# adelacvg/detail_tts

Measured on AMD Instinct MI355X. Metric: generated audio seconds/sec (24 kHz), 10 s prompt, batch 8 per GPU, higher is better.
Workload: dtype f32; 1 GPU; configs[2]: 1xMI355X batch-8, 10 s prompts (T_ref=936), 234 codes -> 9.984 s audio per utterance; GPT KV-cache decode + 50-step CFG diffusion + flow-VAE/HiFiGAN vocoder, seed-0 random-init weights; batch_per_gpu=8, codes=234, diffusion_steps=50, parallelism=replica x1

## Files before the change

detail_tts_amd/csrc/conv_gemm.h:

```cpp
#pragma once
#include "common.h"

namespace dtts {

struct ConvParams {
    const float* x = nullptr;
    long long x_bs = 0;
    int x_cs = 0;
    const int* len_in = nullptr;
    const int* x_bidx = nullptr;
    int Tin = 0;
    const float* pro_ab = nullptr;
    int pro_act = ACT_NONE;
    float pro_slope = 0.f;
    const float* w = nullptr;
    const float* bias = nullptr;
    int Cin = 0, CinP = 0, Cout = 0, CoutP = 0, KW = 1, stride = 1, dil = 1, pad = 0;
    const float* badd = nullptr;
    int badd_bs = 0;
    int gate = GATE_NONE;
    int epi_act = ACT_NONE;
    float epi_slope = 0.f;
    float out_scale = 1.f;
    const float* res = nullptr;
// ... 22 lines not shown
    int gn_ada_stride = 0;
    const int* gn_ada_idx = nullptr;
    int gn_act = ACT_NONE, gn_groups = 32;
    float gn_eps = 1e-5f;
    void* gn_xch = nullptr;
    unsigned gn_tag = 0;
    int* gn_err = nullptr;
    const int* cols = nullptr;
    int ncols = 0, cols_b0 = 0;
    void* next3 = nullptr;
    int next_c8 = 0, next_tp = 0, next_halo = 0, next_act = ACT_NONE;
    float next_slope = 0.f;
    int* next_sat = nullptr;
    int ksplit = 1;
    int ksplit_max = 0;
    int p1 = 0;
    int epi_vec = 0;
    float* kpart = nullptr;
    int* kcount = nullptr;
    int ablate = 0;
};

void launch_conv_gemm(const ConvParams& p, hipStream_t stream);
void set_conv_small_tiles(int n);

}
```

detail_tts_amd/csrc/conv_gemm.hip:

```cpp
#include <atomic>
#include <cstdlib>
#include "conv_gemm_kernel.h"

namespace dtts {

static int conv_small_tiles_default() {
    static const int n = env_int("DTTS_CONV_SMALL_TILES", 384);
    return n;
}
static std::atomic<int> g_conv_small_tiles{-1};
void set_conv_small_tiles(int n) { g_conv_small_tiles.store(n < 0 ? -1 : n, std::memory_order_relaxed); }

void launch_conv_gemm(const ConvParams& p_in, hipStream_t stream) {
    static const int ablate = env_int("DTTS_CONV_ABLATE", 0);
    ConvParams p = p_in;
    p.ablate = ablate;
    DTTS_REQUIRE(p.B > 0 && p.Nout > 0 && p.Cout > 0 && p.Cin > 0, "empty conv");
    DTTS_REQUIRE(p.x && p.w && p.y, "null pointer");
    DTTS_REQUIRE(p.gate == GATE_NONE || p.phases == 1, "gate+phases unsupported");
    const int halo = (p.KW - 1) * p.dil;
    auto fits = [&](int bn) { return (bn - 1) * p.stride + halo + 1 <= XW_MAX; };
    const int small_opt = g_conv_small_tiles.load(std::memory_order_relaxed);
    const int small_tiles = small_opt >= 0 ? small_opt : conv_small_tiles_default();
    if (small_tiles > 0 && p.CoutP % 64 == 0 && fits(64) && (long long)cdiv(p.CoutP, 128) * cdiv(p.Nout, 128) * p.B <= small_tiles) {
        static const int small_bk = env_int("DTTS_CONV_SMALL_BK", 32);
        if (small_bk == 32 && p.CinP % 32 == 0 && p.KW * p.dil <= 3) launch_conv_tile<64, 64, 2, 2, 32>(p, stream, "conv_gemm_kernel<64,64,k32>");
        else launch_conv_tile<64, 64, 2, 2, 16>(p, stream, "conv_gemm_kernel<64,64,k16>");
        return;
    }
    if (p.CoutP % 128 == 0) {
        const int pad128 = round_up(p.Nout, 128), pad64 = round_up(p.Nout, 64);
        if (fits(128) && (pad128 - pad64) * 10 <= p.Nout) {
            launch_conv_tile<128, 128, 2, 2, 16>(p, stream, "conv_gemm_kernel<128,128,k16>");
        } else {
            DTTS_REQUIRE(fits(64), "conv halo too large");
            launch_conv_tile<128, 64, 2, 2, 16>(p, stream, "conv_gemm_kernel<128,64,k16>");
        }
    } else if (p.CoutP % 64 == 0) {
        if (fits(128) && p.Nout > 64) launch_conv_tile<64, 128, 2, 2, 16>(p, stream, "conv_gemm_kernel<64,128,k16>");
// ... 10 lines not shown
```

detail_tts_amd/csrc/conv_x3.h:

```cpp
#pragma once
#include "conv_gemm.h"

namespace dtts {

constexpr int X3_HALO = 1;
constexpr int X3_BN = 192;
static inline int x3_tp(int T) { return round_up(T, X3_BN) + 2 * X3_HALO; }
static inline size_t x3_bytes(int B, int C, int T) { return (size_t)B * (C / 8) * 2 * x3_tp(T) * 16; }

void launch_split_weights(const float* wp, int KW, int CinP, int CoutP, void* out, hipStream_t s);
void launch_split_planes(const float* x, long long x_bs, int x_cs, const float* ab, int act, const int* lens, int T, int B, int C,
                         void* out, hipStream_t s);
void launch_split_planes_taps(const float* x, long long x_bs, int x_cs, const int* lens, int T, int B, int C, int KW, int pad, void* out,
                              hipStream_t s, int* sat = nullptr);
void launch_gn_split_planes(const float* x, long long x_bs, int x_cs, const int* lens, int T, int B, int C, int groups,
                            const float* gamma, const float* beta, float eps, const float* ada, int ada_stride, int ada_bs, int act,
                            void* out, hipStream_t s, const int* ada_idx = nullptr);
void launch_conv_x3(const ConvParams& p, hipStream_t s);

constexpr size_t X3_SLAB_FLOATS = 96 * 256, X3_MAX_SLABS = 1024, X3_SPLIT_COUNTERS = 4096;
void x3_split_workspace(hipStream_t s, size_t nslabs, float** part, int** count);

constexpr int GN_FUSE_MAX_NT = 6;
size_t conv_x3_gn_xch_bytes(int B, int Cout, int T);
bool conv_x3_gn_fusable(int Cout, int CoutP, int Cin, int KW, int groups, int B, int T);

constexpr int X3D_HALO = 32;
static inline int x3d_tp(int T) { return round_up(T, X3_BN) + 64 + X3D_HALO; }
static inline size_t x3d_bytes(int B, int CP, int T) { return (size_t)B * (CP / 8) * 2 * x3d_tp(T) * 16; }
void launch_split_planes_ex(const float* x, long long x_bs, int x_cs, int act, float slope, const int* lens, int T, int B, int C, int CP,
                            int halo, int Tp, void* out, hipStream_t s, int* sat = nullptr);
void launch_conv_x3d(const ConvParams& p, hipStream_t s);
void launch_zero_plane_margins(const int* lens, int T, int B, int CP, int halo, int Tp, void* out, hipStream_t s);
// ... 3 lines not shown
```

detail_tts_amd/csrc/conv_x3.hip:

```cpp
#include <algorithm>
#include <cstdio>
#include <mutex>
#include <type_traits>
#include <utility>
#include <vector>

#include "conv_x3.h"
#include <cstdlib>
#include "prof.h"
#include "split3.h"

namespace dtts {

typedef float f32x16 __attribute__((ext_vector_type(16)));

namespace {
constexpr int NPL = XS_PLANES, NK = 2 * NPL;
constexpr int BM = 128, BN = X3_BN;
constexpr int WTILE = NK * BM * 16;
constexpr int XMAIN = NK * BN * 16;
constexpr int XBUF = XMAIN + NK * 2 * 16;
typedef unsigned gn_u4 __attribute__((ext_vector_type(4)));
constexpr int GN_AUX_SC1 = 16;
constexpr int GN_MAXW = 8;
// ... 37 lines not shown
        }
#pragma unroll
        for (int e = 0; e < 8; ++e) v[e] *= XS_SCALE_X;
        split8(v, q0, q1);
    }
    uint4* o = out + ((long long)(b * C8 + c8) * NPL) * Tp + tp;
    o[0] = q0;
    o[Tp] = q1;
}

template <int ACT>
__global__ __launch_bounds__(1024) void gn_split_planes_kernel(const float* __restrict__ x, long long x_bs, int x_cs,
                                                              const int* __restrict__ lens, int T, int C, int groups,
                                                              const float* __restrict__ gamma, const float* __restrict__ beta, float eps,
                                                              const float* __restrict__ ada, int ada_stride, int ada_bs, int Tp,
                                                              uint4* __restrict__ out, const int* __restrict__ ada_idx) {
    __shared__ float red[2][16];
    __shared__ float sa[64], sd[64];
    const int g = blockIdx.x, b = blockIdx.y, tid = threadIdx.x, lane = tid & 63, wave = tid >> 6, nthr = blockDim.x;
    const int len = lens ? lens[b] : T;
    const int cpg = C / groups;
    const float* xg = x + (long long)b * x_bs + (long long)(g * cpg) * x_cs;
    const float k = xg[0];
    float s1 = 0.f, s2 = 0.f;
    const bool vec = ((x_cs & 3) == 0) && ((reinterpret_cast<unsigned long long>(xg) & 15ull) == 0);
    if (vec) {
        const int len4 = len >> 2, n4 = cpg * len4;
        for (int i0 = tid; i0 < n4; i0 += 4 * nthr) {
            float4 v[4];
#pragma unroll
            for (int u = 0; u < 4; ++u) {
                const int i = i0 + u * nthr, ic = i < n4 ? i : 0;
                const int row = ic / len4, t4 = ic - row * len4;
                v[u] = reinterpret_cast<const float4*>(xg + (long long)row * x_cs)[t4];
            }
#pragma unroll
            for (int u = 0; u < 4; ++u) {
// ... 61 lines not shown
                v[e] *= XS_SCALE_X;
            }
            split8(v, q0, q1);
        }
        uint4* o = out + ((long long)(b * C8 + g * c8n + c8l) * NPL) * Tp + tp;
        o[0] = q0;
        o[Tp] = q1;
    }
}

template <int ACT, int NI>
__global__ __launch_bounds__(1024) void gn_split_planes_reg_kernel(const float* __restrict__ x, long long x_bs, int x_cs,
                                                                  const int* __restrict__ lens, int T, int C, int groups,
                                                                  const float* __restrict__ gamma, const float* __restrict__ beta, float eps,
                                                                  const float* __restrict__ ada, int ada_stride, int ada_bs, int Tp,
                                                                  uint4* __restrict__ out, const int* __restrict__ ada_idx) {
    __shared__ float red[2][16];
    __shared__ float sa[64], sd[64];
    const int g = blockIdx.x, b = blockIdx.y, tid = threadIdx.x, lane = tid & 63, wave = tid >> 6;
    const int len = lens ? lens[b] : T;
    const int cpg = C / groups, c8n = cpg >> 3, C8 = C >> 3, nitems = c8n * Tp;
    const float* xg = x + (long long)b * x_bs + (long long)(g * cpg) * x_cs;
    const float k = xg[0];
    float v[NI][8];
    float s1 = 0.f, s2 = 0.f;
#pragma unroll
    for (int q = 0; q < NI; ++q) {
        const int item = tid + q * 1024, c8l = item / Tp, t = item - c8l * Tp - X3_HALO;
        const bool ok = item < nitems && t >= 0 && t < len;
        const float* xr = xg + (long long)(ok ? c8l * 8 : 0) * x_cs + (ok ? t : 0);
#pragma unroll
        for (int e = 0; e < 8; ++e) v[q][e] = xr[(long long)e * x_cs];
        if (ok) {
            float d[8];
#pragma unroll
            for (int e = 0; e < 8; ++e) d[e] = v[q][e] - k;
            s1 += ((d[0] + d[1]) + (d[2] + d[3])) + ((d[4] + d[5]) + (d[6] + d[7]));
// ... 846 lines not shown
    uint4* o = static_cast<uint4*>(out);
    const double n = (double)B * C * T;
    ProfScope ps("split_planes_kernel", 0.0, n * 8.0, s);
    if (ab) {
        if (act == ACT_SILU) hipLaunchKernelGGL((split_planes_kernel<ACT_SILU, true>), grid, dim3(256), 0, s, x, x_bs, x_cs, ab, lens, T, C / 8, Tp, o);
        else hipLaunchKernelGGL((split_planes_kernel<ACT_NONE, true>), grid, dim3(256), 0, s, x, x_bs, x_cs, ab, lens, T, C / 8, Tp, o);
    } else {
        if (act == ACT_SILU) hipLaunchKernelGGL((split_planes_kernel<ACT_SILU, false>), grid, dim3(256), 0, s, x, x_bs, x_cs, ab, lens, T, C / 8, Tp, o);
        else hipLaunchKernelGGL((split_planes_kernel<ACT_NONE, false>), grid, dim3(256), 0, s, x, x_bs, x_cs, ab, lens, T, C / 8, Tp, o);
    }
    DTTS_CHECK_HIP(hipGetLastError());
}

void launch_gn_split_planes(const float* x, long long x_bs, int x_cs, const int* lens, int T, int B, int C, int groups,
                            const float* gamma, const float* beta, float eps, const float* ada, int ada_stride, int ada_bs, int act,
                            void* out, hipStream_t s, const int* ada_idx) {
    DTTS_REQUIRE(C % groups == 0 && (C / groups) % 8 == 0 && C / groups <= 64, "gn_split_planes: group size");
    DTTS_REQUIRE(act == ACT_NONE || act == ACT_SILU, "gn_split_planes: activation");
    const int Tp = x3_tp(T);
    uint4* o = static_cast<uint4*>(out);
    ProfScope ps("gn_split_planes_kernel", 0.0, (double)B * C * T * 8.0, s);
    static const int ns = env_int("DTTS_GN_SPLIT_NS", 1);
    static const int nt = env_int("DTTS_GN_SPLIT_NT", 1024);
    static const bool reg_ok = env_on("DTTS_GN_SPLIT_REG");
    constexpr int NI = 3;
    if (reg_ok && ns == 1 && (C / groups / 8) * Tp <= NI * 1024) {
        if (act == ACT_SILU)
            hipLaunchKernelGGL((gn_split_planes_reg_kernel<ACT_SILU, NI>), dim3(groups, B), dim3(1024), 0, s, x, x_bs, x_cs, lens, T, C, groups,
                               gamma, beta, eps, ada, ada_stride, ada_bs, Tp, o, ada_idx);
        else
            hipLaunchKernelGGL((gn_split_planes_reg_kernel<ACT_NONE, NI>), dim3(groups, B), dim3(1024), 0, s, x, x_bs, x_cs, lens, T, C, groups,
                               gamma, beta, eps, ada, ada_stride, ada_bs, Tp, o, ada_idx);
        DTTS_CHECK_HIP(hipGetLastError());
        return;
    }
    if (act == ACT_SILU)
        hipLaunchKernelGGL(gn_split_planes_kernel<ACT_SILU>, dim3(groups, B, ns), dim3(nt), 0, s, x, x_bs, x_cs, lens, T, C, groups, gamma,
                           beta, eps, ada, ada_stride, ada_bs, Tp, o, ada_idx);
    else
        hipLaunchKernelGGL(gn_split_planes_kernel<ACT_NONE>, dim3(groups, B, ns), dim3(nt), 0, s, x, x_bs, x_cs, lens, T, C, groups, gamma,
                           beta, eps, ada, ada_stride, ada_bs, Tp, o, ada_idx);
    DTTS_CHECK_HIP(hipGetLastError());
}

namespace {
struct KSplitWs {
    float* part;
    int* count;
};
KSplitWs ksplit_workspace(hipStream_t s, size_t nslabs) {
    constexpr int SLOTS = 8;
    constexpr size_t MAX_SLABS = X3_MAX_SLABS, MAX_TILES = X3_SPLIT_COUNTERS;
    static std::mutex mu;
    static hipStream_t owner[SLOTS];
    static int owner_dev[SLOTS];
    static float* part[SLOTS];
// ... 28 lines not shown
}

void x3_split_workspace(hipStream_t s, size_t nslabs, float** part, int** count) {
    const KSplitWs w = ksplit_workspace(s, nslabs);
    *part = w.part;
    *count = w.count;
}

size_t conv_x3_gn_xch_bytes(int B, int Cout, int T) { return (size_t)B * (Cout / 8) * cdiv(T, BN) * 2 * 16; }

static long long split_tiles_max() {
    static const long long v = env_int("DTTS_CONV_KSPLIT_MAXTILE", 128);
    return v;
}

bool conv_x3_gn_fusable(int Cout, int CoutP, int Cin, int KW, int groups, int B, int T) {
    if (Cout != CoutP || Cout % BM || groups <= 0 || Cout % groups || Cout / groups != 24 || Cin % 16 || (KW != 1 && KW != 3)) return false;
    const int nt = cdiv(T, BN);
    (void)B;
    return nt <= GN_FUSE_MAX_NT;
}

void launch_conv_x3(const ConvParams& p_in, hipStream_t s) {
    ConvParams p = p_in;
    DTTS_REQUIRE(p.w3 && p.x3 && (p.y || p.qkv_planes || p.gn_out3) && p.x3_tp > 0, "conv_x3: operands");
    const bool gn = p.gn_out3 != nullptr;
    static const int env_ablate = env_int("DTTS_CONV_ABLATE", 0);
    if (env_ablate) p.ablate = env_ablate;
    if (gn) {
        DTTS_REQUIRE(conv_x3_gn_fusable(p.Cout, p.CoutP, p.Cin, p.KW, p.gn_groups, p.B, p.Nout), "conv_x3: this launch cannot carry a fused GroupNorm");
// ... 6 lines not shown
    DTTS_REQUIRE(p.Cin % 16 == 0 && p.CoutP % BM == 0, "conv_x3: channel padding");
    const bool p1 = p.p1 != 0;
    DTTS_REQUIRE(!p1 || (p.Cin % 32 == 0 && p.gate == GATE_NONE), "conv_x3 one-product mode: input channels a multiple of 32, no gate");
    const bool gated = p.gate == GATE_TANH_SIGMOID;
    DTTS_REQUIRE(p.stride == 1 && p.dil == 1 && p.phases == 1 && (p.gate == GATE_NONE ? !p.badd : gated), "conv_x3: unsupported conv form");
    DTTS_REQUIRE(!gated || (p.KW == 1 && !gn && !p.qkv_planes && !p.res && p.epi_act == ACT_NONE && p.out_scale == 1.f && p.Cout % 2 == 0),
                 "conv_x3 gated epilogue: 1x1 conv, no residual / activation");
    DTTS_REQUIRE((p.KW == 1 && p.pad == 0) || (p.KW == 3 && p.pad == 1), "conv_x3: k = 1 or k = 3 (same padding) only");
    DTTS_REQUIRE(round_up(p.Nout, BN) + 2 * X3_HALO <= p.x3_tp, "conv_x3: time padding");
    static const int force_stg = []() { const int n = env_int("DTTS_CONV_STAGES", 0); return n >= 2 && n <= 4 ? n : 0; }();
    static const long long max3 = env_int("DTTS_CONV_STAGES3_MAXWG", 600);
    static const long long max4 = env_int("DTTS_CONV_STAGES4_MAXWG", 128);
    if (gn) p.cols = nullptr;
    DTTS_REQUIRE(!p.cols || (p.ncols > 0 && p.ncols <= cdiv(p.Nout, BN) * p.B && cdiv(p.Nout, BN) < 256), "conv_x3: column table");
    const long long ntile = (long long)(p.CoutP / BM) * (p.cols ? p.ncols : cdiv(p.Nout, BN) * p.B);
    static const int max_split = []() { const int n = env_int("DTTS_CONV_KSPLIT", 4); return n < 1 ? 1 : (n > 8 ? 8 : n); }();
    int S = 1;
    const long long split_tiles = split_tiles_max();
    static const long long split_wgs = env_int("DTTS_CONV_KSPLIT_WGS", 256);
    const long long ntile_pad = (long long)(p.CoutP / BM) * cdiv(p.Nout, BN) * p.B;
    static const int max_split_k1 = env_int("DTTS_CONV_KSPLIT_K1", 2);
    if (ntile_pad <= split_tiles) S = (int)std::min<long long>(std::min<long long>(p.KW == 3 ? max_split : std::min(max_split, max_split_k1), split_wgs / ntile_pad), (p.Cin >> 4) / 8);
    if (p.ksplit_max > 0) S = std::min(S, p.ksplit_max);
    if (S < 1) S = 1;
    p.ksplit = S;
    static const bool epi_vec_on = env_on("DTTS_X3_EPI_VEC");
    auto al16 = [](const void* q, long long bs, int cs) { return (reinterpret_cast<unsigned long long>(q) & 15ull) == 0 && (bs & 3) == 0 && (cs & 3) == 0; };
    p.epi_vec = (epi_vec_on && p.y && al16(p.y, p.y_bs, p.y_cs) && (!p.res || al16(p.res, p.res_bs, p.res_cs))) ? 1 : 0;
    if (S > 1) {
        const KSplitWs w = ksplit_workspace(s, (size_t)ntile * S);
        p.kpart = w.part;
        p.kcount = w.count;
    }
    const long long nwg = ntile * S;
    static const long long max4k3 = env_int("DTTS_CONV_STAGES4_MAXWG_K3", 128);
    const int nstg = force_stg ? force_stg : (nwg <= (p.KW == 3 ? max4k3 : max4) ? 4 : (nwg <= max3 ? 3 : 2));
    const size_t lds = (size_t)nstg * (WTILE + XBUF) + BM * sizeof(float) + 16 + (gn ? 2 * BM * sizeof(float) : 0);
// ... 54 lines not shown
```

detail_tts_amd/csrc/model.h:

```cpp
#pragma once
#include <map>
#include <memory>
#include <atomic>
#include <thread>
#include <cstring>
#include <memory>
#include <mutex>
#include <string>
#include <unordered_map>
#include <vector>

#include "attention.h"
#include "common.h"
#include "conv_gemm.h"
#include "conv_x3.h"
#include "diff_schedule.h"
#include "gpt_kernels.h"
#include "ops.h"
#include "../../include/detail_hip.h"

namespace dtts {

struct PackedConv {
    const float* w = nullptr;
// ... 203 lines not shown
        else if (key == "gpt_token_min_rows") { DTTS_REQUIRE(value == 1 || value == 4 || value == 8, "gpt_token_min_rows: 1, 4 or 8"); opt_tok_min_rows_ = value; gpt_drop_graphs(); }
        else if (key == "gpt_token_wgs") { DTTS_REQUIRE(value == 128 || value == 64 || value == 32, "gpt_token_wgs: 128, 64 or 32"); opt_tok_wgs_ = value; gpt_drop_graphs(); }
        else if (key == "gpt_token_fault") opt_tok_fault_ = value;
        else if (key == "gpt_token_fault_eos") opt_tok_fault_eos_ = value;
        else if (key == "cfg_streams") opt_cfg_streams_ = value < 0 ? 0 : value;
        else if (key == "gn_fuse") opt_gn_fuse_ = value != 0;
        else if (key == "conv_cols") opt_conv_cols_ = value != 0;
        else if (key == "voc_chain_planes") opt_voc_chain_ = value != 0;
        else if (key == "voc_x3") opt_voc_x3_ = value != 0;
        else if (key == "x3_fault") opt_x3_fault_ = value;
        else if (key == "attn_ksplit_cus") set_attn_ksplit_cus(value);
        else if (key == "attn_ksplit") set_attn_ksplit(value);
        else if (key == "ln_reg") set_ln_channels_reg(value != 0);
        else if (key == "conv_small_tiles") set_conv_small_tiles(value);
        else if (key == "integ_pipeline") opt_integ_pipeline_ = value;
        else throw Error(-1, "unknown option '" + key + "'");
    }
    int get_option(const std::string& key) const {
        if (key == "conv_x3") return use_x3() ? 1 : 0;
        if (key == "trunk_fp16") return opt_trunk_fp16_ ? 1 : 0;
        throw Error(-1, "option '" + key + "' cannot be read back");
    }
    std::string last_error;
    dtts_config cfg;
    int device;

private:
    friend struct Stage;
    const float* W(const std::string& name, size_t numel) const;
    const float* Wopt(const std::string& name, size_t numel) const;
// ... 48 lines not shown
    };
    struct TrunkIo {
        const int* lens;
        int B, T, Ta;
        hipStream_t s;
        float* ab;
        void* xs = nullptr;
        GnFuse* f = nullptr;
        bool p1 = false;
        const int* step_idx = nullptr;
    };
    void norm_input(const float* x, int C, const float* gamma, const float* beta, int act, bool x3, const TrunkIo& io);
    void attention_block(const AttnBlockW& w, const float* x, float* y, float* qkv, float* att, const TrunkIo& io, const GnNext* next = nullptr);
    void res_block_fwd(const Schedule& sc, const ResBlockW& w, const float* x, float* h1, float* y, int step, const TrunkIo& io,
                       const GnNext* next = nullptr);
    struct GnXch {
        void* buf = nullptr;
        size_t bytes = 0;
        unsigned tag = 0;
    };
    static constexpr int GN_SLOTS = 8;
    GnXch gn_xch_[GN_SLOTS];
    int* gn_err_host_ = nullptr;
    int* gn_err_dev_ = nullptr;
    bool opt_gn_fuse_ = false;
    void gn_fill(ConvParams& p, int slot, size_t bytes, const GnNext& n, void* out3, int groups, hipStream_t s);
    void gn_check();
    bool use_x3() const;
    void diff_forward_pair(const Schedule& sc, const float* x, const float* cbuf0, const int* lens2, const int* lens_i, const int* umap, int B, int Nu,
                           int T, int step, float* out2, hipStream_t s, const float* integ = nullptr);
// ... 98 lines not shown
        ~SatScope() { --m->x3_sat_depth_; }
        void check() { if (m->x3_sat_depth_ == 1) m->x3_sat_check(s); }
        SatScope(const SatScope&) = delete;
        SatScope& operator=(const SatScope&) = delete;
    };
    void vocoder_check(long long ticket);
private:
    int opt_cfg_streams_ = 0;
    bool opt_conv_x3_ = true;
    bool opt_trunk_fp16_ = false;
    Arena w3_;
    Arena w3_voc_;
    static constexpr int MAX_CFG_STREAMS = 4;
    hipStream_t sx_[MAX_CFG_STREAMS - 1] = {nullptr, nullptr, nullptr};
    hipEvent_t ev_fork_ = nullptr, ev_joinx_[MAX_CFG_STREAMS - 1] = {nullptr, nullptr, nullptr};
    int opt_integ_pipeline_ = 0;
    hipStream_t si_ = nullptr;
    std::vector<hipEvent_t> ev_integ_;

    bool has_frontend_ = false;
    PackedConv fe_dft_, fe_mel_;
    int fe_nfft_ = 0;

    bool has_vq_ = false;
    MelStyleW vq_ref_enc_;
    PackedConv vq_up1_, vq_up2_, vq_out_;
    const float *vq_table_ = nullptr, *vq_ln_g_ = nullptr, *vq_ln_b_ = nullptr;
    bool has_vq_enc_ = false;
    PackedConv vqe_c1_, vqe_c2_, vqe_c3_, vq_proj_in_;
    const float *vqe_ln_g_ = nullptr, *vqe_ln_b_ = nullptr, *vq_embed_ = nullptr, *vq_embed_sq_ = nullptr;
// ... 26 lines not shown
```

detail_tts_amd/csrc/model_diffusion.hip:

```cpp
#include "model.h"
#include <algorithm>
#include <cmath>
#include <cstring>
#include "prof.h"

namespace dtts {

static void make_masked_stream(hipStream_t* st, int cus) {
    uint32_t mask[8] = {0, 0, 0, 0, 0, 0, 0, 0};
    for (int b = 0; b < cus; ++b) mask[b >> 5] |= 1u << (b & 31);
    DTTS_CHECK_HIP(hipExtStreamCreateWithCUMask(st, 8, mask));
}

static void make_side_stream(hipStream_t* st) {
    static const int reserve = env_int("DTTS_B_CU_RESERVE", 0);
    if (reserve > 0 && reserve < 256) make_masked_stream(st, 256 - reserve);
    else DTTS_CHECK_HIP(hipStreamCreateWithFlags(st, hipStreamNonBlocking));
}

void Model::ensure_fork_events() {
    if (ev_fork_) return;
    DTTS_CHECK_HIP(hipEventCreateWithFlags(&ev_fork_, hipEventDisableTiming));
    for (auto& e : ev_joinx_) DTTS_CHECK_HIP(hipEventCreateWithFlags(&e, hipEventDisableTiming));
}
// ... 313 lines not shown
void Model::res_block_fwd(const Schedule& sc, const ResBlockW& w, const float* x, float* h1, float* y, int step, const TrunkIo& io,
                          const GnNext* next) {
    const int C = cfg.diff_channels, B = io.B, T = io.T, Ta = io.Ta, groups = gn_groups(C);
    const long long bs = (long long)C * Ta;
    GnFuse* f = io.f;
    const bool x3 = io.xs && w.c1.w3 && w.c2.w3;
    DTTS_REQUIRE(!f || x3, "fused GroupNorm needs the split-precision path");
    norm_input(x, C, w.gn1_g, w.gn1_b, ACT_SILU, x3, io);
    ConvParams p = cp(x, C, h1, C, B, T, Ta, io.lens);
    p.pro_ab = io.ab;
    p.pro_act = ACT_SILU;
    if (x3) {
        with_planes(p, io.xs, T);
        p.p1 = io.p1;
    }
    const float* ada = sc.ss_table + (size_t)w.index * 2 * C * sc.n + (io.step_idx ? 0 : step);
    if (f) {
        GnNext n2;
        n2.gamma = w.gn2_g;
        n2.beta = w.gn2_b;
        n2.act = ACT_SILU;
        ConvParams pf = p;
        pf.y = nullptr;
        gn_fill(pf, f->slot, conv_x3_gn_xch_bytes(B, C, T), n2, f->xs_alt, groups, io.s);
        pf.gn_ada = ada;
        pf.gn_ada_stride = sc.n;
        pf.gn_ada_idx = io.step_idx;
        run_conv(w.c1, pf, io.s);
    } else {
        run_conv(w.c1, p, io.s);
        if (x3) launch_gn_split_planes(h1, bs, Ta, io.lens, T, B, C, groups, w.gn2_g, w.gn2_b, 1e-5f, ada, sc.n, 0, ACT_SILU, io.xs, io.s, io.step_idx);
        else launch_gn_coeffs(h1, bs, Ta, io.lens, T, B, C, groups, w.gn2_g, w.gn2_b, 1e-5f, ada, sc.n, 0, io.ab, io.s, io.step_idx);
    }
    ConvParams q = p;
    q.x = h1;
    q.pad = 1;
    q.y = y;
    with_res(q, x, bs, Ta);
    if (f) {
        q.x3 = f->xs_alt;
        if (next) {
            gn_fill(q, f->slot, conv_x3_gn_xch_bytes(B, C, T), *next, io.xs, groups, io.s);
            f->in_ready = true;
        }
    }
    run_conv(w.c2, q, io.s);
}

Model::PairPlan Model::plan_pair(const int* lens_host, int B, int T, hipStream_t s) {
    std::vector<int> l2(2 * B), li, um(2 * B), ul;
    for (int b = 0; b < B; ++b) {
        const int len = lens_host ? lens_host[b] : T;
        l2[b] = l2[B + b] = len;
        li.push_back(len);
        um[b] = b;
        int gidx = -1;
        for (size_t k = 0; k < ul.size(); ++k)
            if (ul[k] == len) gidx = (int)k;
        if (gidx < 0) { gidx = (int)ul.size(); ul.push_back(len); }
        um[B + b] = B + gidx;
// ... 137 lines not shown
        }
        norm_input(cur, C, out_gn_g_, out_gn_b_, ACT_SILU, x3, io);
        ConvParams o = cp(cur, C, T, Ta, lens, out2 + (size_t)b0 * OC * T, OC, T, T, lens, n);
        o.pro_ab = io.ab;
        o.pro_act = ACT_SILU;
        o.pad = 1;
        if (x3) with_planes(o, io.xs, T);
        run_conv(out_conv_, o, st);
    }
    for (int k = 1; k < NS; ++k) {
        DTTS_CHECK_HIP(hipEventRecord(ev_joinx_[k - 1], sx_[k - 1]));
        DTTS_CHECK_HIP(hipStreamWaitEvent(s, ev_joinx_[k - 1], 0));
    }
}

static size_t integ_ws_bytes(int Bv, int C, int T) {
    const size_t act = (size_t)Bv * C * T;
    return sizeof(float) * (act + 2 * (3 * act + qkv_floats(Bv, C, T) + (size_t)2 * Bv * C)) + 2 * x3_bytes(Bv, C, T) + 32 * 256;
}
static int integ_chunk(int Bi) {
    static const int target = env_int("DTTS_INTEG_SAMPLES", 36);
    return std::max(1, target / Bi);
}

void Model::precompute_integrator(const Schedule& sc, const float* cbuf0, const int* lens_i_host, int B, int Nu, int T, const std::vector<int>& steps,
                                  float* integ_all, hipStream_t s, std::vector<std::pair<int, hipEvent_t>>* ready) {
    const int C = cfg.diff_channels, Bi = B + Nu, J = integ_chunk(Bi), NS = (int)steps.size();
    const size_t ct = (size_t)C * T, mark = ws().mark();
    const int Bv = J * Bi;
    const bool x3 = use_x3();
    static const bool env_two = env_on("DTTS_TWO_STREAMS");
    const bool piped = ready != nullptr && NS > J;
    const bool two = (env_two && opt_two_streams_) || piped;
// ... 6 lines not shown
                static const bool low = []() { const char* v = env_str("DTTS_INTEG_PRIO"); return v && v[0] == 'l'; }();
                int least = 0, greatest = 0;
                DTTS_CHECK_HIP(hipDeviceGetStreamPriorityRange(&least, &greatest));
                DTTS_CHECK_HIP(hipStreamCreateWithPriority(&si_, hipStreamNonBlocking, low ? least : 0));
            }
        }
        while ((int)ev_integ_.size() < cdiv(NS, J)) {
            hipEvent_t e;
            DTTS_CHECK_HIP(hipEventCreateWithFlags(&e, hipEventDisableTiming));
            ev_integ_.push_back(e);
        }
    }
    hipStream_t side = piped ? si_ : sx_[0];
    if (two && !piped && !sx_[0]) { make_side_stream(&sx_[0]); side = sx_[0]; }
    if (two) ensure_fork_events();
    float* vin = ws().f32((size_t)Bv * ct);
    for (int j = 0; j < J; ++j)
        DTTS_CHECK_HIP(hipMemcpyAsync(vin + (size_t)j * Bi * ct, cbuf0, sizeof(float) * (size_t)Bi * ct, hipMemcpyDeviceToDevice, s));
    struct Lane { hipStream_t st; float *bufA, *bufB, *bufC, *qkv, *ab; void* xs; };
    Lane lanes[2];
    for (int q = 0; q < (two ? 2 : 1); ++q) {
        lanes[q].st = q ? side : s;
        lanes[q].bufB = ws().f32((size_t)Bv * ct);
        lanes[q].bufC = ws().f32((size_t)Bv * ct);
        lanes[q].bufA = ws().f32((size_t)Bv * ct);
        lanes[q].qkv = ws().f32(qkv_floats(Bv, C, T));
        lanes[q].ab = ws().f32((size_t)2 * Bv * C);
        lanes[q].xs = x3 ? ws().raw(x3_bytes(Bv, C, T)) : nullptr;
    }
    if (two) {
        DTTS_CHECK_HIP(hipEventRecord(ev_fork_, s));
        DTTS_CHECK_HIP(hipStreamWaitEvent(side, ev_fork_, 0));
    }
    std::vector<int> lv(Bv), sv(Bv);
    int ci = 0;
    const int prof_rot = prof_rot_++;
    for (int k0 = 0; k0 < NS; k0 += J, ++ci) {
        const Lane& L = lanes[piped ? (ci ? 1 : 0) : (two ? (ci & 1) : 0)];
        Profiler::gate() = ((ci / 2 + prof_rot) % Profiler::get().step_every) == 0;
        const int jn = std::min(J, NS - k0), nb = jn * Bi;
        for (int j = 0; j < jn; ++j)
            for (int b = 0; b < Bi; ++b) {
                lv[j * Bi + b] = lens_i_host[b];
                sv[j * Bi + b] = steps[k0 + j];
            }
        const int* dl = upload_ints(lv.data(), nb, L.st);
        const int* ds = upload_ints(sv.data(), nb, L.st);
        register_cols(dl, lv.data(), nb, T, L.st);
        float* outp = integ_all + (size_t)k0 * Bi * ct;
        TrunkIo io{dl, nb, T, T, L.st, L.ab};
        io.xs = L.xs;
        io.step_idx = ds;
        auto dlayer = [&](const DiffLayerW& l, const float* in, float* o) {
            res_block_fwd(sc, l.rb, in, L.bufB, L.bufC, 0, io);
            attention_block(l.at, L.bufC, o, L.qkv, L.bufB, io);
        };
        dlayer(integ_[0], vin, L.bufA);
        dlayer(integ_[1], L.bufA, L.bufA);
        dlayer(integ_[2], L.bufA, outp);
        register_cols(dl, nullptr, 0, T, L.st);
        if (piped && ci) {
            DTTS_CHECK_HIP(hipEventRecord(ev_integ_[ci], si_));
            ready->emplace_back(k0, ev_integ_[ci]);
        }
    }
    Profiler::gate() = true;
    if (piped) return;
    if (two) {
        DTTS_CHECK_HIP(hipEventRecord(ev_joinx_[0], sx_[0]));
        DTTS_CHECK_HIP(hipStreamWaitEvent(s, ev_joinx_[0], 0));
    }
    ws().rewind(mark);
// ... 86 lines not shown
    gn_check();
    DTTS_REQUIRE(bound_, "weights not bound");
    DTTS_REQUIRE(sampler == 0 || sampler == 1 || sampler == 2, "sampler: 0 (p), 1 (ddim) or 2 (dpmsolver++)");
    DTTS_REQUIRE(eta >= 0.f, "eta must be >= 0");
    Schedule& sc = schedule(sched_id);
    const bool dpm = sampler == 2;
    DTTS_REQUIRE(dpm == (sc.kind == 1), dpm ? "sampler 2 (dpmsolver++) runs on a DPM schedule (dtts_diff_schedule_dpm)"
                                            : "samplers 0 / 1 run on an integer-timestep schedule (dtts_diff_schedule)");
    DTTS_REQUIRE(!dpm || (eta == 0.f && !step_noise), "dpmsolver++ draws no noise: eta must be 0 and step_noise NULL");
    const int C = cfg.diff_channels, OC = cfg.diff_out_channels, MC = cfg.mel_channels;
    if (n_steps <= 0 || n_steps > sc.n) n_steps = sc.n;
    static const bool env_pre_on = env_on("DTTS_INTEG_PRECOMPUTE");
    static const double max_gb = []() { const char* v = env_str("DTTS_INTEG_MAX_GB"); return v ? atof(v) : 24.0; }();
    const size_t integ_table = sizeof(float) * (size_t)n_steps * 2 * B * C * T;
    const bool env_pre = env_pre_on && (double)integ_table <= max_gb * 1073741824.0;
    const size_t integ_bytes = env_pre ? integ_table + integ_ws_bytes(integ_chunk(B + 1) * 2 * B, C, T) : 0;
    const size_t hist_floats = dpm ? (size_t)B * MC * T : 0;
    const PairCall pc = begin_pair(code_emb, lens_host, sample_ids_host, B, T, s, integ_bytes, hist_floats);
    const PairPlan& pl = pc.pl;
    const int *lens2 = pl.lens2, *sids = pc.sids;
    float *cbuf0 = pc.cbuf0, *out2 = pc.out2, *x0_hist = pc.hist;
    float* x = mel_out;
    const long long xbs = (long long)MC * T;
    if (x_init) {
        DTTS_CHECK_HIP(hipMemcpyAsync(x, x_init, sizeof(float) * (size_t)B * MC * T, hipMemcpyDeviceToDevice, s));
    } else {
        DTTS_CHECK_HIP(hipMemsetAsync(x, 0, sizeof(float) * (size_t)B * MC * T, s));
        for (int b = 0; b < B; ++b) {
            const int len = lens_host ? lens_host[b] : T;
            if (len == T) {
                launch_philox_normal(x + (size_t)b * xbs, xbs, MC * T, 1, seed, sids + b, STAGE_DIFF_INIT, 0, 1.f, s);
// ... 211 lines not shown
```

detail_tts_amd/csrc/ops.h:

```cpp
#pragma once
#include "common.h"

namespace dtts {

void launch_gn_coeffs(const float* x, long long x_bs, int x_cs, const int* lens, int T, int B, int C, int groups,
                      const float* gamma, const float* beta, float eps, const float* ada, int ada_stride, int ada_bs,
                      float* ab_out, hipStream_t s, const int* ada_idx = nullptr);

void launch_affine_apply(const float* x, long long x_bs, int x_cs, const float* ab, const int* lens, int T, int B, int C,
                         int up, int act, float* y, long long y_bs, int y_cs, hipStream_t s);

void set_ln_channels_reg(bool on);
void launch_ln_channels(const float* x, const float* r, long long bs, int cs, const int* lens, int T, int B, int C,
                        const float* gamma, const float* beta, float eps, float* y, long long y_bs, int y_cs, hipStream_t s);

void launch_mean_time(const float* x, long long x_bs, int x_cs, const int* lens, int T, int B, int C, float* out, hipStream_t s);

void launch_broadcast_channels(const float* v, int B, int C, int T, float* y, long long y_bs, int y_cs, hipStream_t s);

void launch_timestep_sinusoid(const int* ts, int n, int dim, float* out, hipStream_t s);
void launch_timestep_sinusoid(const float* ts, int n, int dim, float* out, hipStream_t s);

void launch_philox_normal(float* out, long long bs, int n, int B, unsigned long long seed, const int* sample_ids, int stage,
                          int step, float scale, hipStream_t s);
// ... 63 lines not shown
```

detail_tts_amd/csrc/ops.hip:

```cpp
#include <atomic>
#include "ops.h"
#include "philox.h"

namespace dtts {

__device__ __forceinline__ float wave_sum(float v) {
#pragma unroll
    for (int o = 32; o > 0; o >>= 1) v += __shfl_xor(v, o);
    return v;
}

__device__ __forceinline__ float block_sum(float v, float* red) {
    v = wave_sum(v);
    const int lane = threadIdx.x & 63, wave = threadIdx.x >> 6;
    __syncthreads();
    if (lane == 0) red[wave] = v;
    __syncthreads();
    float t = 0.f;
    for (int i = 0; i < (int)(blockDim.x >> 6); ++i) t += red[i];
    return t;
}

__global__ __launch_bounds__(256) void gn_coeffs_kernel(const float* x, long long x_bs, int x_cs, const int* lens, int T, int C,
                                                        int groups, const float* gamma, const float* beta, float eps,
                                                        const float* ada, int ada_stride, int ada_bs, float* ab_out, const int* ada_idx) {
    __shared__ float red[8];
    const int g = blockIdx.x, b = blockIdx.y;
    const int len = lens ? lens[b] : T;
    const int cpg = C / groups;
    const float* xg = x + (long long)b * x_bs + (long long)(g * cpg) * x_cs;
    const int n = cpg * len;
    const float k = xg[0];
    float s1 = 0.f, s2 = 0.f;
    const bool vec = ((x_cs & 3) == 0) && ((reinterpret_cast<unsigned long long>(xg) & 15ull) == 0);
    if (vec) {
        const int len4 = len >> 2;
        int c = 0;
        for (; c + 8 <= cpg; c += 8) {
            for (int t = threadIdx.x; t < len4; t += blockDim.x) {
                float4 v[8];
#pragma unroll
                for (int u = 0; u < 8; ++u) v[u] = reinterpret_cast<const float4*>(xg + (long long)(c + u) * x_cs)[t];
#pragma unroll
                for (int u = 0; u < 8; ++u) {
                    const float d0 = v[u].x - k, d1 = v[u].y - k, d2 = v[u].z - k, d3 = v[u].w - k;
// ... 36 lines not shown
        float d = beta[c] - mean * a;
        if (ada) {
            const float* ad = ada + (ada_idx ? (long long)ada_idx[b] : (long long)b * ada_bs);
            const float sc = 1.f + ad[(long long)c * ada_stride], sh = ad[(long long)(C + c) * ada_stride];
            a *= sc;
            d = d * sc + sh;
        }
        float* o = ab_out + ((long long)b * C + c) * 2;
        o[0] = a;
        o[1] = d;
    }
}

void launch_gn_coeffs(const float* x, long long x_bs, int x_cs, const int* lens, int T, int B, int C, int groups,
                      const float* gamma, const float* beta, float eps, const float* ada, int ada_stride, int ada_bs,
                      float* ab_out, hipStream_t s, const int* ada_idx) {
    DTTS_REQUIRE(C % groups == 0 && C / groups <= 256, "group size");
    hipLaunchKernelGGL(gn_coeffs_kernel, dim3(groups, B), dim3(256), 0, s, x, x_bs, x_cs, lens, T, C, groups, gamma, beta, eps,
                       ada, ada_stride, ada_bs, ab_out, ada_idx);
    DTTS_CHECK_HIP(hipGetLastError());
}

__global__ void affine_apply_kernel(const float* x, long long x_bs, int x_cs, const float* ab, const int* lens, int T, int C,
                                    int up, int act, float* y, long long y_bs, int y_cs) {
    const int c = blockIdx.y, b = blockIdx.z;
    const int len = (lens ? lens[b] : T) * up;
    const float a = ab ? ab[((long long)b * C + c) * 2] : 1.f, d = ab ? ab[((long long)b * C + c) * 2 + 1] : 0.f;
    const float* xr = x + (long long)b * x_bs + (long long)c * x_cs;
    float* yr = y + (long long)b * y_bs + (long long)c * y_cs;
    for (int t = blockIdx.x * blockDim.x + threadIdx.x; t < len; t += gridDim.x * blockDim.x)
        yr[t] = act_apply(a * xr[t / up] + d, act, 0.f);
}

void launch_affine_apply(const float* x, long long x_bs, int x_cs, const float* ab, const int* lens, int T, int B, int C,
// ... 393 lines not shown
```

Baseline: 179.4 audio_s/s.

## Share first integ res-block conv1 across replicated step samples

New measurement: 180.2 audio_s/s, median of 6. No clear change (+0.4%).

```diff
diff --git a/detail_tts_amd/csrc/conv_gemm.h b/detail_tts_amd/csrc/conv_gemm.h
--- a/detail_tts_amd/csrc/conv_gemm.h
+++ b/detail_tts_amd/csrc/conv_gemm.h
@@ -60,6 +60,7 @@
     int* next_sat = nullptr;
     int ksplit = 1;
     int ksplit_max = 0;
+    int rule_B = 0;
     int p1 = 0;
     int epi_vec = 0;
     float* kpart = nullptr;
@@ -68,6 +69,7 @@
 };
 
 void launch_conv_gemm(const ConvParams& p, hipStream_t stream);
+bool conv_gemm_small_launch(int CoutP, int Nout, int B);
 void set_conv_small_tiles(int n);
 
 }
diff --git a/detail_tts_amd/csrc/conv_gemm.hip b/detail_tts_amd/csrc/conv_gemm.hip
--- a/detail_tts_amd/csrc/conv_gemm.hip
+++ b/detail_tts_amd/csrc/conv_gemm.hip
@@ -11,6 +11,15 @@
 static std::atomic<int> g_conv_small_tiles{-1};
 void set_conv_small_tiles(int n) { g_conv_small_tiles.store(n < 0 ? -1 : n, std::memory_order_relaxed); }
 
+static int conv_small_tiles_now() {
+    const int small_opt = g_conv_small_tiles.load(std::memory_order_relaxed);
+    return small_opt >= 0 ? small_opt : conv_small_tiles_default();
+}
+bool conv_gemm_small_launch(int CoutP, int Nout, int B) {
+    const int small_tiles = conv_small_tiles_now();
+    return small_tiles > 0 && CoutP % 64 == 0 && (long long)cdiv(CoutP, 128) * cdiv(Nout, 128) * B <= small_tiles;
+}
+
 void launch_conv_gemm(const ConvParams& p_in, hipStream_t stream) {
     static const int ablate = env_int("DTTS_CONV_ABLATE", 0);
     ConvParams p = p_in;
@@ -20,9 +29,7 @@
     DTTS_REQUIRE(p.gate == GATE_NONE || p.phases == 1, "gate+phases unsupported");
     const int halo = (p.KW - 1) * p.dil;
     auto fits = [&](int bn) { return (bn - 1) * p.stride + halo + 1 <= XW_MAX; };
-    const int small_opt = g_conv_small_tiles.load(std::memory_order_relaxed);
-    const int small_tiles = small_opt >= 0 ? small_opt : conv_small_tiles_default();
-    if (small_tiles > 0 && p.CoutP % 64 == 0 && fits(64) && (long long)cdiv(p.CoutP, 128) * cdiv(p.Nout, 128) * p.B <= small_tiles) {
+    if (fits(64) && conv_gemm_small_launch(p.CoutP, p.Nout, p.rule_B > 0 ? p.rule_B : p.B)) {
         static const int small_bk = env_int("DTTS_CONV_SMALL_BK", 32);
         if (small_bk == 32 && p.CinP % 32 == 0 && p.KW * p.dil <= 3) launch_conv_tile<64, 64, 2, 2, 32>(p, stream, "conv_gemm_kernel<64,64,k32>");
         else launch_conv_tile<64, 64, 2, 2, 16>(p, stream, "conv_gemm_kernel<64,64,k16>");
diff --git a/detail_tts_amd/csrc/conv_x3.h b/detail_tts_amd/csrc/conv_x3.h
--- a/detail_tts_amd/csrc/conv_x3.h
+++ b/detail_tts_amd/csrc/conv_x3.h
@@ -15,8 +15,9 @@
                               hipStream_t s, int* sat = nullptr);
 void launch_gn_split_planes(const float* x, long long x_bs, int x_cs, const int* lens, int T, int B, int C, int groups,
                             const float* gamma, const float* beta, float eps, const float* ada, int ada_stride, int ada_bs, int act,
-                            void* out, hipStream_t s, const int* ada_idx = nullptr);
+                            void* out, hipStream_t s, const int* ada_idx = nullptr, int x_bmod = 0);
 void launch_conv_x3(const ConvParams& p, hipStream_t s);
+int conv_x3_ksplit(int KW, int Cin, int CoutP, int Nout, int B);
 
 constexpr size_t X3_SLAB_FLOATS = 96 * 256, X3_MAX_SLABS = 1024, X3_SPLIT_COUNTERS = 4096;
 void x3_split_workspace(hipStream_t s, size_t nslabs, float** part, int** count);
diff --git a/detail_tts_amd/csrc/conv_x3.hip b/detail_tts_amd/csrc/conv_x3.hip
--- a/detail_tts_amd/csrc/conv_x3.hip
+++ b/detail_tts_amd/csrc/conv_x3.hip
@@ -75,13 +75,13 @@
                                                               const int* __restrict__ lens, int T, int C, int groups,
                                                               const float* __restrict__ gamma, const float* __restrict__ beta, float eps,
                                                               const float* __restrict__ ada, int ada_stride, int ada_bs, int Tp,
-                                                              uint4* __restrict__ out, const int* __restrict__ ada_idx) {
+                                                              uint4* __restrict__ out, const int* __restrict__ ada_idx, int x_bmod) {
     __shared__ float red[2][16];
     __shared__ float sa[64], sd[64];
     const int g = blockIdx.x, b = blockIdx.y, tid = threadIdx.x, lane = tid & 63, wave = tid >> 6, nthr = blockDim.x;
     const int len = lens ? lens[b] : T;
     const int cpg = C / groups;
-    const float* xg = x + (long long)b * x_bs + (long long)(g * cpg) * x_cs;
+    const float* xg = x + (long long)(x_bmod ? b % x_bmod : b) * x_bs + (long long)(g * cpg) * x_cs;
     const float k = xg[0];
     float s1 = 0.f, s2 = 0.f;
     const bool vec = ((x_cs & 3) == 0) && ((reinterpret_cast<unsigned long long>(xg) & 15ull) == 0);
@@ -173,13 +173,13 @@
                                                                   const int* __restrict__ lens, int T, int C, int groups,
                                                                   const float* __restrict__ gamma, const float* __restrict__ beta, float eps,
                                                                   const float* __restrict__ ada, int ada_stride, int ada_bs, int Tp,
-                                                                  uint4* __restrict__ out, const int* __restrict__ ada_idx) {
+                                                                  uint4* __restrict__ out, const int* __restrict__ ada_idx, int x_bmod) {
     __shared__ float red[2][16];
     __shared__ float sa[64], sd[64];
     const int g = blockIdx.x, b = blockIdx.y, tid = threadIdx.x, lane = tid & 63, wave = tid >> 6;
     const int len = lens ? lens[b] : T;
     const int cpg = C / groups, c8n = cpg >> 3, C8 = C >> 3, nitems = c8n * Tp;
-    const float* xg = x + (long long)b * x_bs + (long long)(g * cpg) * x_cs;
+    const float* xg = x + (long long)(x_bmod ? b % x_bmod : b) * x_bs + (long long)(g * cpg) * x_cs;
     const float k = xg[0];
     float v[NI][8];
     float s1 = 0.f, s2 = 0.f;
@@ -1056,9 +1056,10 @@
 
 void launch_gn_split_planes(const float* x, long long x_bs, int x_cs, const int* lens, int T, int B, int C, int groups,
                             const float* gamma, const float* beta, float eps, const float* ada, int ada_stride, int ada_bs, int act,
-                            void* out, hipStream_t s, const int* ada_idx) {
+                            void* out, hipStream_t s, const int* ada_idx, int x_bmod) {
     DTTS_REQUIRE(C % groups == 0 && (C / groups) % 8 == 0 && C / groups <= 64, "gn_split_planes: group size");
     DTTS_REQUIRE(act == ACT_NONE || act == ACT_SILU, "gn_split_planes: activation");
+    DTTS_REQUIRE(x_bmod >= 0, "gn_split_planes: shared input");
     const int Tp = x3_tp(T);
     uint4* o = static_cast<uint4*>(out);
     ProfScope ps("gn_split_planes_kernel", 0.0, (double)B * C * T * 8.0, s);
@@ -1069,19 +1070,19 @@
     if (reg_ok && ns == 1 && (C / groups / 8) * Tp <= NI * 1024) {
         if (act == ACT_SILU)
             hipLaunchKernelGGL((gn_split_planes_reg_kernel<ACT_SILU, NI>), dim3(groups, B), dim3(1024), 0, s, x, x_bs, x_cs, lens, T, C, groups,
-                               gamma, beta, eps, ada, ada_stride, ada_bs, Tp, o, ada_idx);
+                               gamma, beta, eps, ada, ada_stride, ada_bs, Tp, o, ada_idx, x_bmod);
         else
             hipLaunchKernelGGL((gn_split_planes_reg_kernel<ACT_NONE, NI>), dim3(groups, B), dim3(1024), 0, s, x, x_bs, x_cs, lens, T, C, groups,
-                               gamma, beta, eps, ada, ada_stride, ada_bs, Tp, o, ada_idx);
+                               gamma, beta, eps, ada, ada_stride, ada_bs, Tp, o, ada_idx, x_bmod);
         DTTS_CHECK_HIP(hipGetLastError());
         return;
     }
     if (act == ACT_SILU)
         hipLaunchKernelGGL(gn_split_planes_kernel<ACT_SILU>, dim3(groups, B, ns), dim3(nt), 0, s, x, x_bs, x_cs, lens, T, C, groups, gamma,
-                           beta, eps, ada, ada_stride, ada_bs, Tp, o, ada_idx);
+                           beta, eps, ada, ada_stride, ada_bs, Tp, o, ada_idx, x_bmod);
     else
         hipLaunchKernelGGL(gn_split_planes_kernel<ACT_NONE>, dim3(groups, B, ns), dim3(nt), 0, s, x, x_bs, x_cs, lens, T, C, groups, gamma,
-                           beta, eps, ada, ada_stride, ada_bs, Tp, o, ada_idx);
+                           beta, eps, ada, ada_stride, ada_bs, Tp, o, ada_idx, x_bmod);
     DTTS_CHECK_HIP(hipGetLastError());
 }
 
@@ -1140,6 +1141,16 @@
     return v;
 }
 
+int conv_x3_ksplit(int KW, int Cin, int CoutP, int Nout, int B) {
+    static const int max_split = []() { const int n = env_int("DTTS_CONV_KSPLIT", 4); return n < 1 ? 1 : (n > 8 ? 8 : n); }();
+    static const long long split_wgs = env_int("DTTS_CONV_KSPLIT_WGS", 256);
+    static const int max_split_k1 = env_int("DTTS_CONV_KSPLIT_K1", 2);
+    const long long ntile_pad = (long long)(CoutP / BM) * cdiv(Nout, BN) * B;
+    int S = 1;
+    if (ntile_pad <= split_tiles_max()) S = (int)std::min<long long>(std::min<long long>(KW == 3 ? max_split : std::min(max_split, max_split_k1), split_wgs / ntile_pad), (Cin >> 4) / 8);
+    return S < 1 ? 1 : S;
+}
+
 bool conv_x3_gn_fusable(int Cout, int CoutP, int Cin, int KW, int groups, int B, int T) {
     if (Cout != CoutP || Cout % BM || groups <= 0 || Cout % groups || Cout / groups != 24 || Cin % 16 || (KW != 1 && KW != 3)) return false;
     const int nt = cdiv(T, BN);
@@ -1176,13 +1187,7 @@
     if (gn) p.cols = nullptr;
     DTTS_REQUIRE(!p.cols || (p.ncols > 0 && p.ncols <= cdiv(p.Nout, BN) * p.B && cdiv(p.Nout, BN) < 256), "conv_x3: column table");
     const long long ntile = (long long)(p.CoutP / BM) * (p.cols ? p.ncols : cdiv(p.Nout, BN) * p.B);
-    static const int max_split = []() { const int n = env_int("DTTS_CONV_KSPLIT", 4); return n < 1 ? 1 : (n > 8 ? 8 : n); }();
-    int S = 1;
-    const long long split_tiles = split_tiles_max();
-    static const long long split_wgs = env_int("DTTS_CONV_KSPLIT_WGS", 256);
-    const long long ntile_pad = (long long)(p.CoutP / BM) * cdiv(p.Nout, BN) * p.B;
-    static const int max_split_k1 = env_int("DTTS_CONV_KSPLIT_K1", 2);
-    if (ntile_pad <= split_tiles) S = (int)std::min<long long>(std::min<long long>(p.KW == 3 ? max_split : std::min(max_split, max_split_k1), split_wgs / ntile_pad), (p.Cin >> 4) / 8);
+    int S = conv_x3_ksplit(p.KW, p.Cin, p.CoutP, p.Nout, p.rule_B > 0 ? p.rule_B : p.B);
     if (p.ksplit_max > 0) S = std::min(S, p.ksplit_max);
     if (S < 1) S = 1;
     p.ksplit = S;
diff --git a/detail_tts_amd/csrc/model.h b/detail_tts_amd/csrc/model.h
--- a/detail_tts_amd/csrc/model.h
+++ b/detail_tts_amd/csrc/model.h
@@ -241,6 +241,7 @@
         else if (key == "ln_reg") set_ln_channels_reg(value != 0);
         else if (key == "conv_small_tiles") set_conv_small_tiles(value);
         else if (key == "integ_pipeline") opt_integ_pipeline_ = value;
+        else if (key == "integ_share") opt_integ_share_ = value != 0;
         else throw Error(-1, "unknown option '" + key + "'");
     }
     int get_option(const std::string& key) const {
@@ -319,6 +320,8 @@
     void attention_block(const AttnBlockW& w, const float* x, float* y, float* qkv, float* att, const TrunkIo& io, const GnNext* next = nullptr);
     void res_block_fwd(const Schedule& sc, const ResBlockW& w, const float* x, float* h1, float* y, int step, const TrunkIo& io,
                        const GnNext* next = nullptr);
+    void res_block_tail(const Schedule& sc, const ResBlockW& w, const float* h1, int h1_bmod, const int* h1_bidx, const float* res,
+                        int res_bmod, float* y, int step, const TrunkIo& io);
     struct GnXch {
         void* buf = nullptr;
         size_t bytes = 0;
@@ -447,6 +450,7 @@
     static constexpr int MAX_CFG_STREAMS = 4;
     hipStream_t sx_[MAX_CFG_STREAMS - 1] = {nullptr, nullptr, nullptr};
     hipEvent_t ev_fork_ = nullptr, ev_joinx_[MAX_CFG_STREAMS - 1] = {nullptr, nullptr, nullptr};
+    bool opt_integ_share_ = true;
     int opt_integ_pipeline_ = 0;
     hipStream_t si_ = nullptr;
     std::vector<hipEvent_t> ev_integ_;
diff --git a/detail_tts_amd/csrc/model_diffusion.hip b/detail_tts_amd/csrc/model_diffusion.hip
--- a/detail_tts_amd/csrc/model_diffusion.hip
+++ b/detail_tts_amd/csrc/model_diffusion.hip
@@ -351,36 +351,57 @@
         with_planes(p, io.xs, T);
         p.p1 = io.p1;
     }
+    if (!f) {
+        run_conv(w.c1, p, io.s);
+        res_block_tail(sc, w, h1, 0, nullptr, x, 0, y, step, io);
+        return;
+    }
     const float* ada = sc.ss_table + (size_t)w.index * 2 * C * sc.n + (io.step_idx ? 0 : step);
-    if (f) {
-        GnNext n2;
-        n2.gamma = w.gn2_g;
-        n2.beta = w.gn2_b;
-        n2.act = ACT_SILU;
-        ConvParams pf = p;
-        pf.y = nullptr;
-        gn_fill(pf, f->slot, conv_x3_gn_xch_bytes(B, C, T), n2, f->xs_alt, groups, io.s);
-        pf.gn_ada = ada;
-        pf.gn_ada_stride = sc.n;
-        pf.gn_ada_idx = io.step_idx;
-        run_conv(w.c1, pf, io.s);
-    } else {
-        run_conv(w.c1, p, io.s);
-        if (x3) launch_gn_split_planes(h1, bs, Ta, io.lens, T, B, C, groups, w.gn2_g, w.gn2_b, 1e-5f, ada, sc.n, 0, ACT_SILU, io.xs, io.s, io.step_idx);
-        else launch_gn_coeffs(h1, bs, Ta, io.lens, T, B, C, groups, w.gn2_g, w.gn2_b, 1e-5f, ada, sc.n, 0, io.ab, io.s, io.step_idx);
-    }
+    GnNext n2;
+    n2.gamma = w.gn2_g;
+    n2.beta = w.gn2_b;
+    n2.act = ACT_SILU;
+    ConvParams pf = p;
+    pf.y = nullptr;
+    gn_fill(pf, f->slot, conv_x3_gn_xch_bytes(B, C, T), n2, f->xs_alt, groups, io.s);
+    pf.gn_ada = ada;
+    pf.gn_ada_stride = sc.n;
+    pf.gn_ada_idx = io.step_idx;
+    run_conv(w.c1, pf, io.s);
     ConvParams q = p;
     q.x = h1;
     q.pad = 1;
     q.y = y;
     with_res(q, x, bs, Ta);
-    if (f) {
-        q.x3 = f->xs_alt;
-        if (next) {
-            gn_fill(q, f->slot, conv_x3_gn_xch_bytes(B, C, T), *next, io.xs, groups, io.s);
-            f->in_ready = true;
-        }
-    }
+    q.x3 = f->xs_alt;
+    if (next) {
+        gn_fill(q, f->slot, conv_x3_gn_xch_bytes(B, C, T), *next, io.xs, groups, io.s);
+        f->in_ready = true;
+    }
+    run_conv(w.c2, q, io.s);
+}
+
+void Model::res_block_tail(const Schedule& sc, const ResBlockW& w, const float* h1, int h1_bmod, const int* h1_bidx, const float* res,
+                           int res_bmod, float* y, int step, const TrunkIo& io) {
+    const int C = cfg.diff_channels, B = io.B, T = io.T, Ta = io.Ta, groups = gn_groups(C);
+    const long long bs = (long long)C * Ta;
+    const bool x3 = io.xs && w.c1.w3 && w.c2.w3;
+    const float* ada = sc.ss_table + (size_t)w.index * 2 * C * sc.n + (io.step_idx ? 0 : step);
+    if (x3) launch_gn_split_planes(h1, bs, Ta, io.lens, T, B, C, groups, w.gn2_g, w.gn2_b, 1e-5f, ada, sc.n, 0, ACT_SILU, io.xs, io.s, io.step_idx, h1_bmod);
+    else launch_gn_coeffs(h1, bs, Ta, io.lens, T, B, C, groups, w.gn2_g, w.gn2_b, 1e-5f, ada, sc.n, 0, io.ab, io.s, io.step_idx, h1_bmod);
+    ConvParams q = cp(h1, C, y, C, B, T, Ta, io.lens);
+    q.pro_ab = io.ab;
+    q.pro_act = ACT_SILU;
+    if (x3) {
+        with_planes(q, io.xs, T);
+        q.p1 = io.p1;
+    } else if (h1_bmod) {
+        DTTS_REQUIRE(h1_bidx, "res_block_tail: the shared h1 needs its sample map on the exact fp32 path");
+        q.x_bidx = h1_bidx;
+    }
+    q.pad = 1;
+    with_res(q, res, bs, Ta);
+    q.res_bmod = res_bmod;
     run_conv(w.c2, q, io.s);
 }
 
@@ -548,9 +569,9 @@
     }
 }
 
-static size_t integ_ws_bytes(int Bv, int C, int T) {
+static size_t integ_ws_bytes(int Bv, int C, int T, size_t share_floats) {
     const size_t act = (size_t)Bv * C * T;
-    return sizeof(float) * (act + 2 * (3 * act + qkv_floats(Bv, C, T) + (size_t)2 * Bv * C)) + 2 * x3_bytes(Bv, C, T) + 32 * 256;
+    return sizeof(float) * ((share_floats ? share_floats : act) + 2 * (3 * act + qkv_floats(Bv, C, T) + (size_t)2 * Bv * C)) + 2 * x3_bytes(Bv, C, T) + 32 * 256;
 }
 static int integ_chunk(int Bi) {
     static const int target = env_int("DTTS_INTEG_SAMPLES", 36);
@@ -587,9 +608,13 @@
     hipStream_t side = piped ? si_ : sx_[0];
     if (two && !piped && !sx_[0]) { make_side_stream(&sx_[0]); side = sx_[0]; }
     if (two) ensure_fork_events();
-    float* vin = ws().f32((size_t)Bv * ct);
-    for (int j = 0; j < J; ++j)
-        DTTS_CHECK_HIP(hipMemcpyAsync(vin + (size_t)j * Bi * ct, cbuf0, sizeof(float) * (size_t)Bi * ct, hipMemcpyDeviceToDevice, s));
+    const bool share = opt_integ_share_;
+    float* vin = nullptr;
+    if (!share) {
+        vin = ws().f32((size_t)Bv * ct);
+        for (int j = 0; j < J; ++j)
+            DTTS_CHECK_HIP(hipMemcpyAsync(vin + (size_t)j * Bi * ct, cbuf0, sizeof(float) * (size_t)Bi * ct, hipMemcpyDeviceToDevice, s));
+    }
     struct Lane { hipStream_t st; float *bufA, *bufB, *bufC, *qkv, *ab; void* xs; };
     Lane lanes[2];
     for (int q = 0; q < (two ? 2 : 1); ++q) {
@@ -601,11 +626,34 @@
         lanes[q].ab = ws().f32((size_t)2 * Bv * C);
         lanes[q].xs = x3 ? ws().raw(x3_bytes(Bv, C, T)) : nullptr;
     }
+    const PackedConv& c1 = integ_[0].rb.c1;
+    auto rule_of = [&](int nb) { return x3 ? conv_x3_ksplit(c1.KW, c1.Cin, c1.CoutP, T, nb) : (conv_gemm_small_launch(c1.CoutP, T, nb) ? 1 : 0); };
+    const int nb_full = std::min(J, NS) * Bi, nb_last = (NS % J ? NS % J : std::min(J, NS)) * Bi;
+    float* h1s[2] = {nullptr, nullptr};
+    if (share) {
+        const int* dli = upload_ints(lens_i_host, Bi, s);
+        register_cols(dli, lens_i_host, Bi, T, s);
+        TrunkIo io0{dli, Bi, T, T, s, lanes[0].ab};
+        io0.xs = lanes[0].xs;
+        const ResBlockW& rb = integ_[0].rb;
+        norm_input(cbuf0, C, rb.gn1_g, rb.gn1_b, ACT_SILU, x3, io0);
+        const int nrules = rule_of(nb_last) != rule_of(nb_full) ? 2 : 1;
+        for (int r = 0; r < nrules; ++r) {
+            h1s[r] = ws().f32((size_t)Bi * ct);
+            ConvParams p = cp(cbuf0, C, h1s[r], C, Bi, T, T, dli);
+            p.pro_ab = io0.ab;
+            p.pro_act = ACT_SILU;
+            if (x3) with_planes(p, io0.xs, T);
+            p.rule_B = r ? nb_last : nb_full;
+            run_conv(c1, p, s);
+        }
+        register_cols(dli, nullptr, 0, T, s);
+    }
     if (two) {
         DTTS_CHECK_HIP(hipEventRecord(ev_fork_, s));
         DTTS_CHECK_HIP(hipStreamWaitEvent(side, ev_fork_, 0));
     }
-    std::vector<int> lv(Bv), sv(Bv);
+    std::vector<int> lv(Bv), sv(Bv), mv(Bv);
     int ci = 0;
     const int prof_rot = prof_rot_++;
     for (int k0 = 0; k0 < NS; k0 += J, ++ci) {
@@ -628,7 +676,18 @@
             res_block_fwd(sc, l.rb, in, L.bufB, L.bufC, 0, io);
             attention_block(l.at, L.bufC, o, L.qkv, L.bufB, io);
         };
-        dlayer(integ_[0], vin, L.bufA);
+        if (share) {
+            const int* dm = nullptr;
+            if (!x3) {
+                for (int v = 0; v < nb; ++v) mv[v] = v % Bi;
+                dm = upload_ints(mv.data(), nb, L.st);
+            }
+            float* h1 = (h1s[1] && nb != nb_full) ? h1s[1] : h1s[0];
+            res_block_tail(sc, integ_[0].rb, h1, Bi, dm, cbuf0, Bi, L.bufC, 0, io);
+            attention_block(integ_[0].at, L.bufC, L.bufA, L.qkv, L.bufB, io);
+        } else {
+            dlayer(integ_[0], vin, L.bufA);
+        }
         dlayer(integ_[1], L.bufA, L.bufA);
         dlayer(integ_[2], L.bufA, outp);
         register_cols(dl, nullptr, 0, T, L.st);
@@ -745,7 +804,7 @@
     static const double max_gb = []() { const char* v = env_str("DTTS_INTEG_MAX_GB"); return v ? atof(v) : 24.0; }();
     const size_t integ_table = sizeof(float) * (size_t)n_steps * 2 * B * C * T;
     const bool env_pre = env_pre_on && (double)integ_table <= max_gb * 1073741824.0;
-    const size_t integ_bytes = env_pre ? integ_table + integ_ws_bytes(integ_chunk(B + 1) * 2 * B, C, T) : 0;
+    const size_t integ_bytes = env_pre ? integ_table + integ_ws_bytes(integ_chunk(B + 1) * 2 * B, C, T, opt_integ_share_ ? (size_t)4 * B * C * T : 0) : 0;
     const size_t hist_floats = dpm ? (size_t)B * MC * T : 0;
     const PairCall pc = begin_pair(code_emb, lens_host, sample_ids_host, B, T, s, integ_bytes, hist_floats);
     const PairPlan& pl = pc.pl;
diff --git a/detail_tts_amd/csrc/ops.h b/detail_tts_amd/csrc/ops.h
--- a/detail_tts_amd/csrc/ops.h
+++ b/detail_tts_amd/csrc/ops.h
@@ -5,7 +5,7 @@
 
 void launch_gn_coeffs(const float* x, long long x_bs, int x_cs, const int* lens, int T, int B, int C, int groups,
                       const float* gamma, const float* beta, float eps, const float* ada, int ada_stride, int ada_bs,
-                      float* ab_out, hipStream_t s, const int* ada_idx = nullptr);
+                      float* ab_out, hipStream_t s, const int* ada_idx = nullptr, int x_bmod = 0);
 
 void launch_affine_apply(const float* x, long long x_bs, int x_cs, const float* ab, const int* lens, int T, int B, int C,
                          int up, int act, float* y, long long y_bs, int y_cs, hipStream_t s);
diff --git a/detail_tts_amd/csrc/ops.hip b/detail_tts_amd/csrc/ops.hip
--- a/detail_tts_amd/csrc/ops.hip
+++ b/detail_tts_amd/csrc/ops.hip
@@ -23,12 +23,13 @@
 
 __global__ __launch_bounds__(256) void gn_coeffs_kernel(const float* x, long long x_bs, int x_cs, const int* lens, int T, int C,
                                                         int groups, const float* gamma, const float* beta, float eps,
-                                                        const float* ada, int ada_stride, int ada_bs, float* ab_out, const int* ada_idx) {
+                                                        const float* ada, int ada_stride, int ada_bs, float* ab_out, const int* ada_idx,
+                                                        int x_bmod) {
     __shared__ float red[8];
     const int g = blockIdx.x, b = blockIdx.y;
     const int len = lens ? lens[b] : T;
     const int cpg = C / groups;
-    const float* xg = x + (long long)b * x_bs + (long long)(g * cpg) * x_cs;
+    const float* xg = x + (long long)(x_bmod ? b % x_bmod : b) * x_bs + (long long)(g * cpg) * x_cs;
     const int n = cpg * len;
     const float k = xg[0];
     float s1 = 0.f, s2 = 0.f;
@@ -95,10 +96,10 @@
 
 void launch_gn_coeffs(const float* x, long long x_bs, int x_cs, const int* lens, int T, int B, int C, int groups,
                       const float* gamma, const float* beta, float eps, const float* ada, int ada_stride, int ada_bs,
-                      float* ab_out, hipStream_t s, const int* ada_idx) {
-    DTTS_REQUIRE(C % groups == 0 && C / groups <= 256, "group size");
+                      float* ab_out, hipStream_t s, const int* ada_idx, int x_bmod) {
+    DTTS_REQUIRE(C % groups == 0 && C / groups <= 256 && x_bmod >= 0, "group size");
     hipLaunchKernelGGL(gn_coeffs_kernel, dim3(groups, B), dim3(256), 0, s, x, x_bs, x_cs, lens, T, C, groups, gamma, beta, eps,
-                       ada, ada_stride, ada_bs, ab_out, ada_idx);
+                       ada, ada_stride, ada_bs, ab_out, ada_idx, x_bmod);
     DTTS_CHECK_HIP(hipGetLastError());
 }
 
```
